# MarSaKi/VLN-BEVBert

Measured on AMD Instinct MI355X. Metric: pretrain_samples_per_sec, higher is better.
Workload: dtype bf16+fp32-residual

## Files before the change

### include/bevbert_hip.h

```cpp
#ifndef BEVBERT_HIP_H
#define BEVBERT_HIP_H

#include <stdint.h>

#ifdef __cplusplus
extern "C" {
#endif

typedef struct ihipStream_t* hipStream_t;

#define BEVBERT_F32 0
#define BEVBERT_BF16 1
#define BEVBERT_F16 2

const char* bevbert_last_error(void);
int bevbert_version(void);
int bevbert_hip_error_reset(void);
const char* bevbert_arch(void);
const char* bevbert_attn_last_path(int backward);

int bevbert_bev_lift_bin(const float* depths, const float* T_c2w, const float* T_w2c, const float* S_w2c,
                         const float* pix_scale, int B, int V, int hw, float depth_scale, int dim, float res,
                         float y_clip, int* cell, int* order, int* cell_start, hipStream_t stream);
int bevbert_bev_bin_points(const float* points, const uint8_t* drop_mask, int B, int P, int dim, float res,
// ... 35 lines not shown
                                const float* gamma, const float* beta, void* y16, float* y32, float* z32, float* mean,
                                float* rstd, int rows, int H, float eps, float drop_p, uint64_t seed, uint64_t offset,
                                hipStream_t stream);
int bevbert_layernorm_res32_bwd(const void* dy16, const float* dy32, const float* z32, const float* mean,
                                const float* rstd, const float* gamma, void* dz, void* dx16, float* dgamma,
                                float* dbeta, float* dbias, float* workspace, int rows, int H, float drop_p, uint64_t seed,
                                uint64_t offset, int accumulate, int dz_dtype,
                                hipStream_t stream);
int64_t bevbert_colsum_workspace_floats(int total_cols);
int bevbert_colsum_partial_rows(int rows);
int bevbert_colsum_finalize(const float* partials, int nblocks, int nwhich, int C, float* out0, float* out1,
                            float* out2, int accumulate, hipStream_t stream);
int bevbert_colsum_partials(const void* dy, float* partials, int rows, int C, int dtype, hipStream_t stream);
int bevbert_multi_finalize(const void* tasks, int ntasks, hipStream_t stream);
int bevbert_multi_accum(const void* tasks, int ntasks, hipStream_t stream);

int bevbert_embed_sum_layernorm_fwd(const int64_t* ids, const void* word, const void* pos, const void* type_row,
                                    const float* gamma, const float* beta, void* y, void* z_out, float* mean,
                                    float* rstd, int rows, int L, int H, float eps, int dtype, float drop_p,
                                    uint64_t seed, uint64_t offset, hipStream_t stream);

int bevbert_embedding_grad(const int64_t* ids, const void* d, float* table_grad, int rows, int H, int padding_idx,
                           int dtype, hipStream_t stream);

int64_t bevbert_smallk_workspace_floats(int rows, int K, int H);
int bevbert_smallk_linear_layernorm_fwd(const float* feat, const float* weight, const float* bias, const float* gamma,
                                        const float* beta, const void* post1, const void* table, const int64_t* idx,
                                        void* y, float* mean, float* rstd, int rows, int K, int H, float eps, int dtype,
                                        hipStream_t stream);
int bevbert_smallk_linear_layernorm_bwd(const void* dy, const float* feat, const float* weight, const float* bias,
// ... 28 lines not shown

int bevbert_bias_gelu_fwd(const void* x, const float* bias, void* y, int rows, int C, int dtype, hipStream_t stream);
int bevbert_bias_gelu_bwd(const void* dy, const void* x, const float* bias, void* dx, float* dbias, float* workspace,
                          int rows, int C, int dtype, int accumulate, hipStream_t stream);
int bevbert_bias_relu_fwd(const void* x, const float* bias, void* y, int rows, int C, int dtype, hipStream_t stream);
int bevbert_bias_relu_bwd(const void* dy, const void* x, const float* bias, void* dx, float* dbias, float* workspace,
                          int rows, int C, int dtype, int accumulate, hipStream_t stream);
int bevbert_colsum(const void* dy, float* out, float* workspace, int rows, int C, int dtype, int accumulate,
                   hipStream_t stream);

int bevbert_segment_wsum(const void* src, const int* rowptr, const int* idx, const float* w, void* out, int out_rows,
                         int H, int dtype, hipStream_t stream);

int bevbert_grad_norm_clip(const float* grads, int64_t n, float pre_scale, float max_norm, float* partials,
                           float* scalars, hipStream_t stream);
int bevbert_adamw_step(float* params, const float* grads, float* exp_avg, float* exp_avg_sq, void* params_bf16,
                       const uint8_t* chunk_flags, int* chunk_steps, int64_t n, const float* grad_scale_dev,
                       const float* lr_dev, float lr, float beta1, float beta2, float eps, float weight_decay,
                       hipStream_t stream);
int bevbert_cast_f32(const float* src, void* dst, int64_t n, int dst_dtype, hipStream_t stream);
int bevbert_zero(void* p, int64_t bytes, hipStream_t stream);
int bevbert_accum_partials(const void* partials, float* sink, int S, int64_t n, int dtype, hipStream_t stream);

int bevbert_gemm(const void* A, const void* B, void* C, const void* bias, int M, int N, int K, int opA, int opB,
                 int64_t lda, int64_t ldb, int64_t ldc, int batch, int64_t stride_a, int64_t stride_b,
                 int64_t stride_c, int in_dtype, int out_dtype, int bias_dtype, float alpha, void* workspace,
                 int64_t workspace_bytes, int autotune, hipStream_t stream);
int bevbert_gemm_plan(int M, int N, int K, int opA, int opB, int64_t lda, int64_t ldb, int64_t ldc, int batch,
                      int64_t stride_a, int64_t stride_b, int64_t stride_c, int in_dtype, int out_dtype, int bias_dtype,
                      int accumulate, int64_t workspace_bytes, int autotune);
// ... 95 lines not shown
```

### vln_bevbert_amd/arena.py

```python
import math

import torch

from . import lib
from .lib import ptr, stream


def call(name, *args):
    from . import ops
    return ops.call(name, *args)

CHUNK = 1024
_ZERO_KERNEL = __import__("os").environ.get("BEVBERT_ZERO_KERNEL", "0") == "1"
NO_DECAY = ("bias", "LayerNorm.bias", "LayerNorm.weight")


def _round_up(n, m):
    return (n + m - 1) // m * m


class ParamArena:
    def __init__(self, module, device, compute_dtype=torch.float32, groups=()):
        self.device = torch.device(device)
        self.compute_dtype = compute_dtype
# ... 42 lines not shown
                self._flags_host[start // CHUNK:end // CHUNK] |= 1
            for n in seg:
                self._seg_of[n] = (start // CHUNK, end // CHUNK)
        self.flags = self._flags_host.to(dev)
        self.chunk_steps = torch.zeros(off // CHUNK, dtype=torch.int32, device=dev)
        self._touched = set()
        self._flags_dirty = False
        self.publish_grads = True
        self.allreduce_group = None
        self.defer_allreduce = False
        self._cb_queued = False
        self._fresh = []
        self._published = []
        self._param_versions = None
        self.step_count = 0
        self._scalars = torch.zeros(4, dtype=torch.float32, device=dev)
        self._partials = torch.zeros(1024, dtype=torch.float32, device=dev)
        self.named = named
        for n, p in named:
            o, k = self.slices[n]
            view = self.params[o:o + k].view(p.shape)
            view.copy_(p.data.to(dev, torch.float32))
            p.data = view
            p.main_grad = self.grads[o:o + k].view(p.shape)
            p.compute = self.shadow[o:o + k].view(p.shape) if self.shadow is not None else p.data
            p.arena = self
            p.arena_name = n
        self._index = {n: i for i, (n, _) in enumerate(named)}
        self.sync_shadow()
        self._param_versions = sum(p._version for _, p in named)

    def packed(self, names, shape):
        o0, _ = self.slices[names[0]]
        total = 0
        for n in names:
            o, k = self.slices[n]
            assert o == o0 + total, f"{names} are not contiguous in the arena"
            total += k
        assert total == math.prod(shape)
        src = self.shadow if self.shadow is not None else self.params
        return src[o0:o0 + total].view(shape), self.grads[o0:o0 + total].view(shape)

    def touch(self, param):
        n = param.arena_name
        if n not in self._touched:
            self._touched.add(n)
            a, b = self._seg_of[n]
            self._flags_host[a:b] |= 2
            self._flags_dirty = True
        if self.publish_grads:
            self._note_backward_write(param)

    def _note_backward_write(self, param):
        if not self._cb_queued:
            try:
                torch.autograd.Variable._execution_engine.queue_callback(self._publish)
            except RuntimeError:
                return
            self._cb_queued = True
# ... 48 lines not shown

    def sync(self):
        if self.device.type == "cuda":
            from . import ops
            ops.WgradStream.flush_all()
            cur = torch.cuda.current_stream(self.device)
            for side in ops.Branches.side_streams():
                if ops.Branches.enabled or side not in ops.WgradStream.streams or ops.WgradStream.dirty:
                    cur.wait_stream(side)
            ops.WgradStream.dirty = False
            ops.WgradStream.release()

    def backward_done(self):
        self.sync()

    def zero_grad(self, overlap=False):
        self.sync()
        if self.device.type == "cuda":
            from . import ops
            ops.RT.scratch.reset()
            if overlap:
                if getattr(self, "_zero_stream", None) is None:
                    from .hwqueues import side_stream
                    self._zero_stream = side_stream(self.device)
                self._zero_stream.wait_stream(torch.cuda.current_stream(self.device))
                with torch.cuda.stream(self._zero_stream):
                    if _ZERO_KERNEL:
                        self.grads.zero_()
                    else:
                        call("bevbert_zero", ptr(self.grads), self.grads.numel() * 4, stream())
                self._zero_pending = True
                return
            call("bevbert_zero", ptr(self.grads), self.grads.numel() * 4, stream())
            return
        self.grads.zero_()

    def wait_zero(self):
        if getattr(self, "_zero_pending", False):
            torch.cuda.current_stream(self.device).wait_stream(self._zero_stream)
            self._zero_pending = False

    def load_state_dict_into(self, module, sd, strict=True):
        out = module.load_state_dict(sd, strict=strict)
        self.sync_shadow()
        return out

    def set_lr(self, lr):
        self._scalars[2:3].fill_(float(lr))
        self._lr_set = True

    def upload_flags(self):
        if self._flags_dirty:
            self.flags.copy_(self._flags_host, non_blocking=True)
            self._flags_dirty = False

    def clip_and_step(self, lr=None, betas=(0.9, 0.98), eps=1e-6, weight_decay=0.01, max_norm=5.0, grad_pre_scale=1.0):
        self.sync()
        if self.exp_avg is None:
            self.exp_avg = torch.zeros_like(self.params)
            self.exp_avg_sq = torch.zeros_like(self.params)
        if lr is not None:
            self.set_lr(lr)
        elif not getattr(self, "_lr_set", False):
            raise RuntimeError("clip_and_step(lr=None) reads the device-resident learning rate: call set_lr() first "
                               "(the slot starts at 0, which would silently turn AdamW and its weight decay into a no-op)")
        if not torch.cuda.is_current_stream_capturing():
            self.upload_flags()
        self.step_count += 1
        call("bevbert_grad_norm_clip", ptr(self.grads), self.numel, float(grad_pre_scale),
             float(max_norm if max_norm is not None else -1.0), ptr(self._partials), ptr(self._scalars), stream())
        call("bevbert_adamw_step", ptr(self.params), ptr(self.grads), ptr(self.exp_avg), ptr(self.exp_avg_sq),
             ptr(self.shadow), ptr(self.flags), ptr(self.chunk_steps), self.numel, self._scalars[1:].data_ptr(),
             self._scalars[2:].data_ptr(), 0.0, float(betas[0]), float(betas[1]), float(eps), float(weight_decay),
             stream())

    def grad_norm(self):
        return self._scalars[0]
```

### vln_bevbert_amd/csrc/capi.hip

```cpp
#include <stdarg.h>

#include "attn_common.h"

static thread_local char g_err[512] = "";

void bb_set_error(const char* fmt, ...) {
  va_list ap;
  va_start(ap, fmt);
  vsnprintf(g_err, sizeof(g_err), fmt, ap);
  va_end(ap);
}

BEVBERT_API const char* bevbert_last_error(void) { return g_err; }
BEVBERT_API int bevbert_hip_error_reset(void) {
  int n = 0;
  while (hipGetLastError() != hipSuccess && n < 16) ++n;
  return n;
}

BEVBERT_API int bevbert_zero(void* p, int64_t bytes, hipStream_t stream) {
  BB_REQUIRE(p != nullptr && bytes >= 0, "zero: null pointer or negative size");
  if (bytes == 0) return BB_OK;
  hipError_t e = hipMemsetAsync(p, 0, (size_t)bytes, stream);
  if (e != hipSuccess) {
    bb_set_error("zero: hipMemsetAsync failed: %s", hipGetErrorString(e));
    return BB_ELAUNCH;
  }
  return BB_OK;
}

BEVBERT_API int bevbert_version(void) { return 112; }

static const uint32_t* g_step_salt = nullptr;
const uint32_t* bb_step_salt() { return g_step_salt; }
BEVBERT_API int bevbert_set_step_salt(const void* device_word) {
  g_step_salt = static_cast<const uint32_t*>(device_word);
  return BB_OK;
}
BEVBERT_API const char* bevbert_arch(void) { return "gfx950"; }

int attn_simple_fwd(const AttnArgs& a, int dtype, hipStream_t st);
int attn_simple_bwd(const AttnArgs& a, int dtype, hipStream_t st);
int attn_delta(const AttnArgs& a, float* delta, int dtype, hipStream_t st);
int attn_mfma_fwd(const AttnArgs& a, hipStream_t st);
int attn_mfma_bwd(const AttnArgs& a, hipStream_t st);
int attn_mfma_bwd1(const AttnArgs& a, hipStream_t st);
// ... 166 lines not shown
```

### vln_bevbert_amd/csrc/rowops.hip

```cpp
#include <math.h>

#include "common.h"

template <typename T, int NV, bool GATHER>
__global__ __launch_bounds__(256) void ln_fwd_kernel(const T* __restrict__ x, const float* __restrict__ bias,
                                                     const T* __restrict__ residual, const float* __restrict__ gamma,
                                                     const float* __restrict__ beta, T* __restrict__ y,
                                                     T* __restrict__ z_out, float* __restrict__ mean_out,
                                                     float* __restrict__ rstd_out, int rows, float eps, float drop_p,
                                                     uint32_t drop_thr, uint32_t drop_key,
                                                     const int64_t* __restrict__ ids, const T* __restrict__ word,
                                                     const T* __restrict__ pos, const T* __restrict__ type_row, int L,
                                                     const uint32_t* __restrict__ salt) {
  constexpr int H = NV * 256;
  if (drop_p > 0.f) drop_key = bb_salted(drop_key, salt);
  const int lane = threadIdx.x & 63;
  const int row = blockIdx.x * 4 + (threadIdx.x >> 6);
  if (row >= rows) return;
  float4 v[NV];
  const float keep_scale = drop_p > 0.f ? 1.0f / (1.0f - drop_p) : 1.0f;
#pragma unroll
  for (int i = 0; i < NV; ++i) {
    const int col = (i * 64 + lane) * 4;
    float4 a;
// ... 502 lines not shown
  for (unsigned i = threadIdx.x; i < t.n4; i += 256) {
    float4 acc = *reinterpret_cast<const float4*>(t.sink + (size_t)i * 4);
    for (int s = 0; s < t.S; ++s) {
      const float4 v = ld4<T>(part + ((size_t)s * t.n4_total + t.off4 + i) * 4);
      acc.x += v.x; acc.y += v.y; acc.z += v.z; acc.w += v.w;
    }
    *reinterpret_cast<float4*>(t.sink + (size_t)i * 4) = acc;
  }
}
__global__ __launch_bounds__(256) void multi_accum_kernel(const AccumTask* __restrict__ tasks) {
  const AccumTask t = tasks[blockIdx.x];
  if (t.dtype == BB_BF16) accum_task<bf16_raw>(t);
  else accum_task<float>(t);
}

#define EG_MAXJ 4
template <typename T, typename TO = float, bool ACCUM = true>
__global__ __launch_bounds__(256) void embedding_grad_kernel(const int64_t* __restrict__ ids, const T* __restrict__ d,
                                                             TO* __restrict__ table_grad, int rows, int H,
                                                             int padding_idx) {
  __shared__ int s_flag;
  __shared__ float s_part[4][256 * EG_MAXJ];
  const int r = blockIdx.x, tid = threadIdx.x, lane = tid & 63, wave = tid >> 6;
  const int64_t id = ids[r];
  if (id == (int64_t)padding_idx) return;
  if (tid == 0) s_flag = 0;
  __syncthreads();
  int hit = 0;
  for (int i = tid; i < r; i += 256) hit |= (ids[i] == id);
  if (hit) s_flag = 1;
// ... 79 lines not shown
    const float4 v = *reinterpret_cast<const float4*>(g + i * 4);
    s += (v.x * v.x + v.y * v.y) + (v.z * v.z + v.w * v.w);
  }
  __shared__ float sh[4];
  s = wave_sum(s);
  if ((threadIdx.x & 63) == 0) sh[threadIdx.x >> 6] = s;
  __syncthreads();
  if (threadIdx.x == 0) partials[blockIdx.x] = (sh[0] + sh[1]) + (sh[2] + sh[3]);
}

__global__ void clip_coef_kernel(const float* __restrict__ partials, int n, float pre_scale, float max_norm,
                                 float* __restrict__ scalars) {
  __shared__ double sh[256];
  double s = 0.0;
  for (int i = threadIdx.x; i < n; i += 256) s += (double)partials[i];
  sh[threadIdx.x] = s;
  __syncthreads();
  for (int o = 128; o > 0; o >>= 1) {
    if (threadIdx.x < o) sh[threadIdx.x] += sh[threadIdx.x + o];
    __syncthreads();
  }
  if (threadIdx.x == 0) {
    const float norm = (float)sqrt(sh[0]) * pre_scale;
    float coef = 1.0f;
    if (max_norm > 0.f) {
      coef = max_norm / (norm + 1e-6f);
      coef = coef < 1.0f ? coef : 1.0f;
    }
    scalars[0] = norm;
    scalars[1] = pre_scale * coef;
// ... 659 lines not shown
    return BB_EUNSUPPORTED;
  }
  BB_CHECK_LAUNCH("colsum_partials");
  return BB_OK;
}

BEVBERT_API int bevbert_multi_accum(const void* tasks, int ntasks, hipStream_t stream) {
  static_assert(sizeof(AccumTask) == 40, "AccumTask is part of the C ABI");
  if (ntasks <= 0) return BB_OK;
  BB_REQUIRE(tasks != nullptr, "multi_accum: null task table");
  hipLaunchKernelGGL(multi_accum_kernel, dim3(ntasks), dim3(256), 0, stream, (const AccumTask*)tasks);
  BB_CHECK_LAUNCH("multi_accum");
  return BB_OK;
}

BEVBERT_API int bevbert_multi_finalize(const void* tasks, int ntasks, hipStream_t stream) {
  static_assert(sizeof(FinalizeTask) == 40, "FinalizeTask is part of the C ABI");
  if (ntasks <= 0) return BB_OK;
  BB_REQUIRE(tasks != nullptr, "multi_finalize: null task table");
  hipLaunchKernelGGL(multi_finalize_kernel, dim3(ntasks), dim3(64, 16), 0, stream, (const FinalizeTask*)tasks);
  BB_CHECK_LAUNCH("multi_finalize");
  return BB_OK;
}

BEVBERT_API int bevbert_segment_wsum(const void* src, const int* rowptr, const int* idx, const float* w, void* out,
                                     int out_rows, int H, int dtype, hipStream_t stream) {
  BB_REQUIRE(H % 4 == 0, "segment_wsum: H=%d must be a multiple of 4", H);
  if (out_rows <= 0) return BB_OK;
  if (dtype == BB_F32)
    hipLaunchKernelGGL(gather_wsum_kernel<float>, dim3(out_rows), dim3(192), 0, stream, (const float*)src, rowptr, idx, w, (float*)out, H);
// ... 97 lines not shown
                       rows, H, rows_per_slice, table_rows);
  else {
    bb_set_error("embedding_grad_sliced: dtype %d unsupported", dtype);
    return BB_EUNSUPPORTED;
  }
  BB_CHECK_LAUNCH("embedding_grad_sliced");
  return BB_OK;
}

BEVBERT_API int bevbert_grad_norm_clip(const float* grads, int64_t n, float pre_scale, float max_norm,
                                       float* partials, float* scalars, hipStream_t stream) {
  BB_REQUIRE(n % 4 == 0, "grad_norm_clip: n must be a multiple of 4");
  hipLaunchKernelGGL(sumsq_kernel, dim3(1024), dim3(256), 0, stream, grads, (size_t)n / 4, partials);
  hipLaunchKernelGGL(clip_coef_kernel, dim3(1), dim3(256), 0, stream, partials, 1024, pre_scale, max_norm, scalars);
  BB_CHECK_LAUNCH("grad_norm_clip");
  return BB_OK;
}

BEVBERT_API int bevbert_adamw_step(float* params, const float* grads, float* exp_avg, float* exp_avg_sq,
                                   void* params_bf16, const uint8_t* chunk_flags, int* chunk_steps, int64_t n,
                                   const float* grad_scale_dev, const float* lr_dev, float lr, float beta1,
                                   float beta2, float eps, float weight_decay, hipStream_t stream) {
  BB_REQUIRE(n % 1024 == 0, "adamw_step: arena length must be a multiple of 1024 elements");
  BB_REQUIRE(chunk_steps != nullptr, "adamw_step: per-chunk step counters are required");
  const size_t nchunks = (size_t)n / 1024;
  hipLaunchKernelGGL(adamw_kernel, dim3(nchunks), dim3(256), 0, stream, params, grads, exp_avg, exp_avg_sq,
                     (bf16_raw*)params_bf16, chunk_flags, chunk_steps, nchunks, grad_scale_dev, lr_dev, lr, beta1, beta2, eps,
                     weight_decay, (float)log2((double)beta1), (float)log2((double)beta2));
  BB_CHECK_LAUNCH("adamw_step");
  return BB_OK;
// ... 45 lines not shown
```

### vln_bevbert_amd/lib.py

```python
import ctypes
import os
import re
import subprocess

import torch

_HERE = os.path.dirname(os.path.abspath(__file__))
LIB_PATH = os.path.join(_HERE, "libbevbert_hip.so")
CSRC = os.path.join(_HERE, "csrc")
EXTRA_FLAGS = {"attn_fwd4.hip": ["-fno-slp-vectorize"]}
SOURCES = ["splat.hip", "rowops.hip", "attn_simple.hip", "attn_f32.hip", "attn_mfma.hip", "attn_bwd1.hip", "attn_fwd2.hip", "attn_fwd4.hip", "attn_bwd2.hip", "attn_bwd3.hip", "attn_small.hip", "attn_short.hip", "smallk.hip", "sap_loss.hip", "graph_nav.hip", "nav_expert.hip", "gemm.hip", "capi.hip"]
HEADER = os.path.join(os.path.dirname(_HERE), "include", "bevbert_hip.h")

F32, BF16, F16 = 0, 1, 2
_DT = {torch.float32: F32, torch.bfloat16: BF16, torch.float16: F16}


class BevBertHipError(RuntimeError):
    pass


def dtype_code(t):
    try:
        return _DT[t.dtype if torch.is_tensor(t) else t]
# ... 67 lines not shown
    "bevbert_smallk_linear_layernorm_bwd": [_P] * 12 + [_I, _I, _I, _I, _P],
    "bevbert_rows_scatter": [_P, _P, _P, _I, _I, _I, _I, _P],
    "bevbert_embedding_grad_sliced": [_P, _P, _P, _I, _I, _I, _I, _I, _P],
    "bevbert_bias_gelu_fwd": [_P, _P, _P, _I, _I, _I, _P],
    "bevbert_bias_gelu_bwd": [_P, _P, _P, _P, _P, _P, _I, _I, _I, _I, _P],
    "bevbert_bias_relu_fwd": [_P, _P, _P, _I, _I, _I, _P],
    "bevbert_bias_relu_bwd": [_P, _P, _P, _P, _P, _P, _I, _I, _I, _I, _P],
    "bevbert_colsum": [_P, _P, _P, _I, _I, _I, _I, _P],
    "bevbert_segment_wsum": [_P, _P, _P, _P, _P, _I, _I, _I, _P],
    "bevbert_grad_norm_clip": [_P, _I64, _F, _F, _P, _P, _P],
    "bevbert_adamw_step": [_P, _P, _P, _P, _P, _P, _P, _I64, _P, _P, _F, _F, _F, _F, _F, _P],
    "bevbert_set_step_salt": [_P],
    "bevbert_colsum_partials": [_P, _P, _I, _I, _I, _P],
    "bevbert_multi_finalize": [_P, _I, _P],
    "bevbert_multi_accum": [_P, _I, _P],
    "bevbert_cast_f32": [_P, _P, _I64, _I, _P],
    "bevbert_zero": [_P, _I64, _P],
    "bevbert_accum_partials": [_P, _P, _I, _I64, _I, _P],
    "bevbert_dropout_keep_mask": [_P, _I64, _F, _U64, _U64, _P],
    "bevbert_gemm": [_P, _P, _P, _P, _I, _I, _I, _I, _I, _I64, _I64, _I64, _I, _I64, _I64, _I64, _I, _I, _I, _F, _P,
                     _I64, _I, _P],
    "bevbert_colsum_finalize": [_P, _I, _I, _I, _P, _P, _P, _I, _P],
    "bevbert_dropout_add": [_P, _P, _P, _I64, _I, _I, _F, _U64, _U64, _P],
    "bevbert_gm_update": [_P] * 10 + [_I, _I, _P, _P, _P],
    "bevbert_gm_nav_vars": [_P] * 7 + [_I, _I, _I] + [_P] * 7,
    "bevbert_gm_bev_select": [_P, _P, _I, _I, _P, _P, _P, _P, _P],
    "bevbert_gm_gather_views": [_P, _P, _P, _P, _I, _I64, _P],
    "bevbert_gm_embed_update": [_P] * 9 + [_I, _I, _I, _I, _P],
    "bevbert_gm_node_embeds": [_P, _P, _P, _P, _P, _I, _I, _I, _P, _P],
    "bevbert_sap_loss_fwd": [_P] * 15 + [_I, _I, _I, _I, _I, _P],
# ... 94 lines not shown
```

### vln_bevbert_amd/ops_reduce.py

```python
import math
import os as _os

import torch

from . import lib
from .lib import stream
from .ops_core import ATTN_BITS, Branches, RT, call


def join_captured_side_streams(extra=()):
    if not torch.cuda.is_available() or not torch.cuda.is_current_stream_capturing():
        return 0
    cur = torch.cuda.current_stream()
    seen, n = {cur.cuda_stream}, 0
    cands = [ATTN_BITS.stream] + list(Branches._streams.values()) + list(WgradStream.streams) + list(extra)
    for st in cands:
        if st is None or st.cuda_stream in seen:
            continue
        seen.add(st.cuda_stream)
        with torch.cuda.stream(st):
            capturing = torch.cuda.is_current_stream_capturing()
        if capturing:
            cur.wait_stream(st)
            n += 1
# ... 182 lines not shown

ScratchRing.INITIAL = int(_os.environ.get("BEVBERT_SCRATCH_INITIAL_MB", "256")) << 20
RT.scratch = SCRATCH


class ReduceQueue:

    jobs = []
    accum_jobs = []
    table_bytes = {}
    producers = {}
    _tables = {}
    _accum_tables = {}
    _dtype = None
    _adtype = None

    @classmethod
    def _note_producer(cls):
        st = WgradStream._target
        if st is None:
            if not torch.cuda.is_available():
                return
            st = torch.cuda.current_stream()
        cls.producers[st.cuda_stream] = st

    @classmethod
    def wait_producers(cls, consumer):
        for h, st in cls.producers.items():
            if h != consumer.cuda_stream:
                consumer.wait_stream(st)
        cls.producers = {}

    @classmethod
    def drop_pending(cls):
        cls.jobs, cls.accum_jobs, cls.producers = [], [], {}

    @classmethod
    def add_accum(cls, partials_ptr, sink_ptr, S, n, dtype):
        cls.accum_jobs.append((partials_ptr, sink_ptr, S, n, dtype))
        cls._note_producer()

    @classmethod
    def _build_accum(cls, jobs, device):
        import numpy as np
        if cls._adtype is None:
            cls._adtype = np.dtype([("partials", "<u8"), ("sink", "<u8"), ("n4_total", "<u8"), ("off4", "<u4"),
                                    ("n4", "<u4"), ("S", "<i4"), ("dtype", "<i4")])
        parts = []
        for partials_ptr, sink_ptr, S, n, dt in jobs:
            n4 = n // 4
            off = np.arange(0, n4, 4096, dtype=np.int64)
            t = np.zeros(len(off), dtype=cls._adtype)
            t["partials"] = partials_ptr
            t["sink"] = sink_ptr + off * 16
            t["n4_total"] = n4
            t["off4"] = off
            t["n4"] = np.minimum(4096, n4 - off)
            t["S"] = S
            t["dtype"] = dt
            parts.append(t)
        table = np.concatenate(parts) if parts else np.zeros(0, dtype=cls._adtype)
        dev = torch.from_numpy(table.view(np.uint8).copy()).to(device)
        cls.table_bytes[dev.data_ptr()] = int(sum(S * n * (4 if dt == lib.F32 else 2) + 8 * n for _, _, S, n, dt in jobs))
        return dev, len(table)

    @classmethod
    def add(cls, partials_ptr, nblocks, nwhich, C, outs, accumulate=1):
        cls.jobs.append((partials_ptr, nblocks, nwhich, C, outs[0] or 0, outs[1] or 0, outs[2] or 0, accumulate))
        cls._note_producer()

    @classmethod
    def _build(cls, jobs, device):
        import numpy as np
        if cls._dtype is None:
            cls._dtype = np.dtype([("partials", "<u8"), ("out", "<u8"), ("nblocks", "<i4"), ("row_stride", "<i4"),
                                   ("col0", "<i4"), ("ncols", "<i4"), ("accumulate", "<i4"), ("pad", "<i4")])
        parts = []
        for partials_ptr, nblocks, nwhich, C, o0, o1, o2, acc in jobs:
            ntile = (C + 63) // 64
# ... 6 lines not shown
                t["out"] = out + tiles * 256
                t["nblocks"] = nblocks
                t["row_stride"] = nwhich * C
                t["col0"] = which * C + tiles * 64
                t["ncols"] = np.minimum(64, C - tiles * 64)
                t["accumulate"] = acc
                parts.append(t)
        table = np.concatenate(parts) if parts else np.zeros(0, dtype=cls._dtype)
        dev = torch.from_numpy(table.view(np.uint8).copy()).to(device)
        cls.table_bytes[dev.data_ptr()] = int(4 * (table["nblocks"].astype(np.int64) * table["ncols"]).sum()
                                              + 4 * (table["ncols"] * (1 + (table["accumulate"] != 0))).sum()) if len(table) else 0
        return dev, len(table)

    @classmethod
    def flush(cls, device):
        if cls.accum_jobs:
            akey = tuple(cls.accum_jobs)
            cls.accum_jobs = []
            aent = cls._accum_tables.get(akey)
            if aent is None:
                if torch.cuda.is_current_stream_capturing():
                    raise lib.BevBertHipError("accumulate task table missing during graph capture (warm-up steps build it)")
                if len(cls._accum_tables) > 256:
                    cls._accum_tables.clear()
                rounds, seen = [[]], [set()]
                for job in akey:
                    r = 0
                    while job[1] in seen[r]:
                        r += 1
                        if r == len(rounds):
                            rounds.append([])
# ... 48 lines not shown
```

### vln_bevbert_amd/train.py

```python
import os
import random

import torch
import torch.distributed as dist

from . import ops
from .static_step import GraphedStep, StaticBatch


def warmup_linear_lr(step, base_lr, warmup_steps, total_steps):
    f = step / warmup_steps if step < warmup_steps else max(0, (total_steps - step) / (total_steps - warmup_steps))
    lr = base_lr * f
    return lr if lr > 0 else 1e-8


def load_gemm_tuning():
    import os
    path = os.path.join(os.path.dirname(os.path.abspath(__file__)), "tunableop_results.csv")
    if os.environ.get("BEVBERT_GEMM_TUNING", "1") != "1" or not os.path.exists(path):
        return 0
    try:
        import torch.cuda.tunable as tunable
        tunable.enable(True)
        tunable.tuning_enable(False)
# ... 215 lines not shown
        first_map = min(arena.slices[n][0] for n in arena.slices
                        if n.startswith("bert.local_encoder") or n.startswith("bert.global_encoder")
                        or not n.startswith("bert."))
        self.reducer = GradReducer(arena.grads, first_map, force=force_collectives)
        self.reducer.set_occupied(arena.slices.values())
        self.reducer.settle_collective_queue()
        self.overlap = overlap and self.reducer.active
        self.capture_ok = not (self.reducer.active and self.reducer.exchange == "bf16_a2a")
        if self.reducer.active and dist.get_backend(self.reducer.group) != "nccl":
            self.capture_ok = False
        if self.reducer.active:
            self.broadcast_state()
        self.early_flush = os.environ.get("BEVBERT_EARLY_FLUSH", "0") == "1" and arena.device.type == "cuda"
        if self.early_flush and not self.overlap:
            model.bert.lang_encoder.register_forward_hook(self._hook_flush)
        if self.overlap:
            self.install_map_layer_hooks()
            model.bert.lang_encoder.register_forward_hook(self._hook_text)
            for k, lo, hi in self.text_layer_regions(model, arena):
                model.bert.lang_encoder.layer[k].register_forward_pre_hook(self._make_layer_hook(lo, hi))

    @staticmethod
    def map_layer_regions(model, arena):
        out = {}
        heads = [(o, o + k) for n, (o, k) in arena.slices.items() if not n.startswith("bert.")]
        if heads:
            lo, hi = min(lo for lo, _ in heads), max(hi for _, hi in heads)
            if not any(n.startswith("bert.") and lo <= o < hi for n, (o, c) in arena.slices.items()):
                out["heads"] = (lo, hi)
        for enc in ("local", "global"):
# ... 85 lines not shown

    def _step_seed(self):
        return (self.seed + self.rank) * 1000003 + self.global_step

    def forward_backward(self, task, batch):
        self.global_step += 1
        ops.RT.new_step(self._step_seed(), plan_key=self._plan_key(task, batch))
        return self._forward_backward(task, batch)

    @staticmethod
    def _plan_key(task, batch):
        return (task, batch.signature) if isinstance(batch, StaticBatch) else None

    def _forward_backward(self, task, batch):
        self._reset_map_hooks()
        self.arena.zero_grad(overlap=self.overlap_zero)
        try:
            if isinstance(batch, StaticBatch):
                loss = self.model.loss_mean(batch.tensors, task)
            else:
                loss = self.model(batch, task, compute_loss=True).mean()
        finally:
            self.arena.wait_zero()
        if self.reducer is not None and self.reducer.timeline is not None:
            self.backward_start = torch.cuda.Event(enable_timing=True)
            self.backward_start.record()
        if loss.is_cuda and loss.dim() == 0:
            one = self.__dict__.get("_one")
            if one is None or one.dtype != loss.dtype or one.device != loss.device:
                one = self._one = torch.ones((), dtype=loss.dtype, device=loss.device)
            loss.backward(gradient=one)
        else:
            loss.backward()
        self.arena.sync()
        self.reducer.finish()
        return loss.detach()

    def optimizer_step(self, lr=None):
        if lr is None:
            lr = warmup_linear_lr(self.global_step, self.lr, self.warmup, self.total)
        self.arena.clip_and_step(lr, self.betas, 1e-6, self.wd, self.grad_norm, grad_pre_scale=1.0 / self.world)

    def step(self, task, batch):
        if isinstance(batch, StaticBatch) and self.use_graphs and self.capture_ok and batch.capturable and ops.RT.trace is None:
            return self._static_step(task, batch)
        loss = self.forward_backward(task, batch)
        self.optimizer_step()
        return loss

    GRAPH_WARMUP = 2

    def _static_step(self, task, sb):
        assert sb.task == task
        self.global_step += 1
        lr = warmup_linear_lr(self.global_step, self.lr, self.warmup, self.total)
        a = self.arena
# ... 22 lines not shown
        torch.cuda.synchronize()
        graph = torch.cuda.CUDAGraph()
        if self._graph_pool is None:
            self._graph_pool = torch.cuda.graph_pool_handle()
        ops.Branches.enabled = branches or self.graph_branches
        mode = "thread_local"
        if self.reducer.active:
            import time
            time.sleep(0.3)
        err = None
        try:
            with torch.cuda.graph(graph, pool=self._graph_pool, capture_error_mode=mode):
                try:
                    ops.RT.new_step(0, write_salt=False, plan_key=self._plan_key(task, sb))
                    loss = self._forward_backward(task, sb)
                    a.clip_and_step(None, self.betas, 1e-6, self.wd, self.grad_norm, grad_pre_scale=1.0 / self.world)
                except Exception as e:
                    err = e
                    ops.join_captured_side_streams(extra=[self.reducer.stream])
        except Exception as e:
            err = err or e
        if err is not None:
            e = err
            import warnings
            self.graph_error = f"{type(e).__name__}: {e}"[:400]
            self.use_graphs = False
            warnings.warn(f"hipGraph capture of the {task} step failed, continuing with eager steps: {self.graph_error}")
            ops.Branches.enabled = branches
            from . import lib
            lib.load().bevbert_hip_error_reset()
            if torch.cuda.is_current_stream_capturing():
# ... 60 lines not shown
```

Measured before the change: 3552.

## Fold grad accumulation into assignment and fuse grad-norm partials into the fold

After: 3599 (median of 6 runs). 1.01x the previous value.

```diff
diff --git a/include/bevbert_hip.h b/include/bevbert_hip.h
--- a/include/bevbert_hip.h
+++ b/include/bevbert_hip.h
@@ -73,6 +73,7 @@
 int bevbert_colsum_partials(const void* dy, float* partials, int rows, int C, int dtype, hipStream_t stream);
 int bevbert_multi_finalize(const void* tasks, int ntasks, hipStream_t stream);
 int bevbert_multi_accum(const void* tasks, int ntasks, hipStream_t stream);
+int bevbert_multi_accum2(const void* tasks, int ntasks, float* sumsq_out, hipStream_t stream);
 
 int bevbert_embed_sum_layernorm_fwd(const int64_t* ids, const void* word, const void* pos, const void* type_row,
                                     const float* gamma, const float* beta, void* y, void* z_out, float* mean,
@@ -131,6 +132,11 @@
 
 int bevbert_grad_norm_clip(const float* grads, int64_t n, float pre_scale, float max_norm, float* partials,
                            float* scalars, hipStream_t stream);
+int bevbert_grad_sumsq_ranges(const float* grads, const void* ranges, int nranges, float* partials_out,
+                              hipStream_t stream);
+int bevbert_zero_ranges(float* grads, const void* ranges, int nranges, hipStream_t stream);
+int bevbert_clip_coef2(const float* sumsq_a, int na, const float* sumsq_b, int nb, float pre_scale, float max_norm,
+                       float* scalars, hipStream_t stream);
 int bevbert_adamw_step(float* params, const float* grads, float* exp_avg, float* exp_avg_sq, void* params_bf16,
                        const uint8_t* chunk_flags, int* chunk_steps, int64_t n, const float* grad_scale_dev,
                        const float* lr_dev, float lr, float beta1, float beta2, float eps, float weight_decay,
diff --git a/vln_bevbert_amd/arena.py b/vln_bevbert_amd/arena.py
--- a/vln_bevbert_amd/arena.py
+++ b/vln_bevbert_amd/arena.py
@@ -80,6 +80,16 @@
         self._published = []
         self._param_versions = None
         self.step_count = 0
+        self.assign_fold = False
+        self._assign_pass = False
+        self._fold_excluded = set()
+        self._touch_count = {}
+        self._fold_plans = {}
+        self._fold_key = None
+        self._fold_state = None
+        self._unzeroed = ()
+        self._range_tables = {}
+        self._slice_starts = None
         self._scalars = torch.zeros(4, dtype=torch.float32, device=dev)
         self._partials = torch.zeros(1024, dtype=torch.float32, device=dev)
         self.named = named
@@ -109,6 +119,8 @@
 
     def touch(self, param):
         n = param.arena_name
+        if self._assign_pass:
+            self._touch_count[n] = self._touch_count.get(n, 0) + 1
         if n not in self._touched:
             self._touched.add(n)
             a, b = self._seg_of[n]
@@ -187,26 +199,124 @@
     def backward_done(self):
         self.sync()
 
-    def zero_grad(self, overlap=False):
+    def zero_grad(self, overlap=False, fold_key=None, assign=False):
         self.sync()
+        self._fold_state = None
+        self._assign_pass = assign = bool(assign) and self.assign_fold
+        self._fold_key = fold_key if assign else None
+        stored = self._fold_plans.get(fold_key) if self._fold_key is not None else None
+        self._unzeroed = stored or ()
+        if assign:
+            self._touch_count.clear()
         if self.device.type == "cuda":
             from . import ops
             ops.RT.scratch.reset()
+            ops.ReduceQueue.begin_pass(self if assign else None)
             if overlap:
                 if getattr(self, "_zero_stream", None) is None:
                     from .hwqueues import side_stream
                     self._zero_stream = side_stream(self.device)
                 self._zero_stream.wait_stream(torch.cuda.current_stream(self.device))
                 with torch.cuda.stream(self._zero_stream):
-                    if _ZERO_KERNEL:
+                    if stored:
+                        self._fill_complement(stored)
+                    elif _ZERO_KERNEL:
                         self.grads.zero_()
                     else:
                         call("bevbert_zero", ptr(self.grads), self.grads.numel() * 4, stream())
                 self._zero_pending = True
                 return
-            call("bevbert_zero", ptr(self.grads), self.grads.numel() * 4, stream())
+            if stored:
+                self._fill_complement(stored)
+            else:
+                call("bevbert_zero", ptr(self.grads), self.grads.numel() * 4, stream())
             return
         self.grads.zero_()
+
+    FOLD_PIECE = 16384
+    MAX_MEMSETS = 16
+
+    def enable_assign_fold(self, module, on=True):
+        self.assign_fold = bool(on) and self.device.type == "cuda"
+        self._fold_state = None
+        if not on:
+            return
+        tables = {id(m.weight) for m in module.modules() if isinstance(m, torch.nn.Embedding)}
+        self._fold_excluded = {n for n, p in self.named if p.dim() != 2 or id(p) in tables or p.shape[1] <= 16}
+        order = sorted((o, k, n) for n, (o, k) in self.slices.items())
+        self._slice_starts = ([o for o, _, _ in order], order)
+
+    def owns_grad_ptr(self, p):
+        return 0 <= p - self.grads.data_ptr() < 4 * self.numel
+
+    def fold_store_flags(self, jobs):
+        import bisect
+        base, starts, order = self.grads.data_ptr(), self._slice_starts[0], self._slice_starts[1]
+        spans = []
+        for _, sink, _, n, _ in jobs:
+            off = (sink - base) // 4
+            spans.append((off, off + n) if (sink - base) % 4 == 0 and 0 <= off and off + n <= self.numel else None)
+        flags, stored = [], []
+        for j, span in enumerate(spans):
+            ok = span is not None and span[0] % CHUNK == 0
+            if ok:
+                lo, hi = span
+                ok = not any(o is not None and i != j and o[0] < _round_up(hi, CHUNK) and lo < o[1]
+                             for i, o in enumerate(spans))
+            if ok:
+                i = bisect.bisect_left(starts, lo)
+                pos, ok = lo, i < len(order) and order[i][0] == lo
+                while ok and pos < hi:
+                    if i == len(order) or order[i][0] != pos:
+                        ok = False
+                        break
+                    o, k, name = order[i]
+                    ok = name not in self._fold_excluded and self._touch_count.get(name, 0) == 1
+                    pos, i = o + k, i + 1
+                ok = ok and pos == hi and (i == len(order) or order[i][0] >= _round_up(hi, CHUNK))
+            flags.append(bool(ok))
+            if ok:
+                stored.append((lo, _round_up(hi, CHUNK)))
+        return tuple(flags), tuple(sorted(stored))
+
+    def fold_ranges(self, stored):
+        ent = self._range_tables.get(stored)
+        if ent is None:
+            if self.device.type == "cuda" and torch.cuda.is_current_stream_capturing():
+                raise lib.BevBertHipError("arena range table missing during graph capture (warm-up steps build it)")
+            if len(self._range_tables) > 64:
+                self._range_tables.clear()
+            merged, pos = [], 0
+            for lo, hi in stored:
+                if lo > pos:
+                    merged.append((pos, lo))
+                pos = max(pos, hi)
+            if pos < self.numel:
+                merged.append((pos, self.numel))
+            pieces = [(a, min(self.FOLD_PIECE, hi - a)) for lo, hi in merged for a in range(lo, hi, self.FOLD_PIECE)]
+            table = torch.tensor(pieces, dtype=torch.int64).reshape(-1, 2).to(self.device)
+            ent = self._range_tables[stored] = {"merged": merged, "table": table, "n": len(pieces),
+                                                "partials": torch.zeros(max(len(pieces), 1), dtype=torch.float32,
+                                                                        device=self.device)}
+        return ent
+
+    def _fill_complement(self, stored):
+        ent = self.fold_ranges(stored)
+        if len(ent["merged"]) <= self.MAX_MEMSETS:
+            for lo, hi in ent["merged"]:
+                call("bevbert_zero", ptr(self.grads) + 4 * lo, 4 * (hi - lo), stream())
+        else:
+            call("bevbert_zero_ranges", ptr(self.grads), ptr(ent["table"]), ent["n"], stream())
+
+    def note_fold(self, stored, sumsq, nstore):
+        if not set(self._unzeroed) <= set(stored):
+            raise lib.BevBertHipError("assign-fold: the step's fill skipped arena ranges its fold did not store "
+                                      f"(plan key {self._fold_key!r} no longer describes the backward pass)")
+        if self._fold_key is not None:
+            if len(self._fold_plans) > 256:
+                self._fold_plans.clear()
+            self._fold_plans[self._fold_key] = stored
+        self._fold_state = (sumsq, nstore, self.fold_ranges(stored))
 
     def wait_zero(self):
         if getattr(self, "_zero_pending", False):
@@ -227,7 +337,8 @@
             self.flags.copy_(self._flags_host, non_blocking=True)
             self._flags_dirty = False
 
-    def clip_and_step(self, lr=None, betas=(0.9, 0.98), eps=1e-6, weight_decay=0.01, max_norm=5.0, grad_pre_scale=1.0):
+    def clip_and_step(self, lr=None, betas=(0.9, 0.98), eps=1e-6, weight_decay=0.01, max_norm=5.0, grad_pre_scale=1.0,
+                      fused_norm=False):
         self.sync()
         if self.exp_avg is None:
             self.exp_avg = torch.zeros_like(self.params)
@@ -240,8 +351,15 @@
         if not torch.cuda.is_current_stream_capturing():
             self.upload_flags()
         self.step_count += 1
-        call("bevbert_grad_norm_clip", ptr(self.grads), self.numel, float(grad_pre_scale),
-             float(max_norm if max_norm is not None else -1.0), ptr(self._partials), ptr(self._scalars), stream())
+        fold, self._fold_state = self._fold_state, None
+        if fused_norm and fold is not None:
+            sumsq, nstore, rt = fold
+            call("bevbert_grad_sumsq_ranges", ptr(self.grads), ptr(rt["table"]), rt["n"], ptr(rt["partials"]), stream())
+            call("bevbert_clip_coef2", ptr(sumsq), nstore, ptr(rt["partials"]), rt["n"], float(grad_pre_scale),
+                 float(max_norm if max_norm is not None else -1.0), ptr(self._scalars), stream())
+        else:
+            call("bevbert_grad_norm_clip", ptr(self.grads), self.numel, float(grad_pre_scale),
+                 float(max_norm if max_norm is not None else -1.0), ptr(self._partials), ptr(self._scalars), stream())
         call("bevbert_adamw_step", ptr(self.params), ptr(self.grads), ptr(self.exp_avg), ptr(self.exp_avg_sq),
              ptr(self.shadow), ptr(self.flags), ptr(self.chunk_steps), self.numel, self._scalars[1:].data_ptr(),
              self._scalars[2:].data_ptr(), 0.0, float(betas[0]), float(betas[1]), float(eps), float(weight_decay),
diff --git a/vln_bevbert_amd/csrc/capi.hip b/vln_bevbert_amd/csrc/capi.hip
--- a/vln_bevbert_amd/csrc/capi.hip
+++ b/vln_bevbert_amd/csrc/capi.hip
@@ -29,7 +29,7 @@
   return BB_OK;
 }
 
-BEVBERT_API int bevbert_version(void) { return 112; }
+BEVBERT_API int bevbert_version(void) { return 113; }
 
 static const uint32_t* g_step_salt = nullptr;
 const uint32_t* bb_step_salt() { return g_step_salt; }
diff --git a/vln_bevbert_amd/csrc/rowops.hip b/vln_bevbert_amd/csrc/rowops.hip
--- a/vln_bevbert_amd/csrc/rowops.hip
+++ b/vln_bevbert_amd/csrc/rowops.hip
@@ -540,6 +540,64 @@
   else accum_task<float>(t);
 }
 
+struct AccumTask2 {
+  const void* partials;
+  float* sink;
+  unsigned long long n4_total;
+  unsigned int off4, n4;
+  int S, dtype;
+  int store, pad;
+};
+template <typename T, bool STORE>
+__device__ __forceinline__ float accum_task2(const AccumTask2& t) {
+  const T* part = (const T*)t.partials + (size_t)t.off4 * 4;
+  const size_t slice = (size_t)t.n4_total * 4;
+  float sq = 0.f;
+  for (unsigned base = threadIdx.x; base < t.n4; base += 1024) {
+    float4 acc[4];
+    bool ok[4];
+#pragma unroll
+    for (int u = 0; u < 4; ++u) {
+      const unsigned i = base + u * 256;
+      ok[u] = i < t.n4;
+      acc[u] = make_float4(0.f, 0.f, 0.f, 0.f);
+      if (!STORE && ok[u]) acc[u] = *reinterpret_cast<const float4*>(t.sink + (size_t)i * 4);
+    }
+    for (int s = 0; s < t.S; ++s) {
+      float4 v[4];
+#pragma unroll
+      for (int u = 0; u < 4; ++u) {
+        const unsigned i = base + u * 256;
+        v[u] = ok[u] ? ld4<T>(part + (size_t)s * slice + (size_t)i * 4) : make_float4(0.f, 0.f, 0.f, 0.f);
+      }
+#pragma unroll
+      for (int u = 0; u < 4; ++u) {
+        acc[u].x += v[u].x; acc[u].y += v[u].y; acc[u].z += v[u].z; acc[u].w += v[u].w;
+      }
+    }
+#pragma unroll
+    for (int u = 0; u < 4; ++u) {
+      if (ok[u]) {
+        *reinterpret_cast<float4*>(t.sink + (size_t)(base + u * 256) * 4) = acc[u];
+        sq += (acc[u].x * acc[u].x + acc[u].y * acc[u].y) + (acc[u].z * acc[u].z + acc[u].w * acc[u].w);
+      }
+    }
+  }
+  return sq;
+}
+__global__ __launch_bounds__(256) void multi_accum2_kernel(const AccumTask2* __restrict__ tasks,
+                                                           float* __restrict__ sumsq_out) {
+  const AccumTask2 t = tasks[blockIdx.x];
+  float sq;
+  if (t.store) sq = t.dtype == BB_BF16 ? accum_task2<bf16_raw, true>(t) : accum_task2<float, true>(t);
+  else sq = t.dtype == BB_BF16 ? accum_task2<bf16_raw, false>(t) : accum_task2<float, false>(t);
+  __shared__ float sh[4];
+  sq = wave_sum(sq);
+  if ((threadIdx.x & 63) == 0) sh[threadIdx.x >> 6] = sq;
+  __syncthreads();
+  if (threadIdx.x == 0) sumsq_out[blockIdx.x] = (sh[0] + sh[1]) + (sh[2] + sh[3]);
+}
+
 #define EG_MAXJ 4
 template <typename T, typename TO = float, bool ACCUM = true>
 __global__ __launch_bounds__(256) void embedding_grad_kernel(const int64_t* __restrict__ ids, const T* __restrict__ d,
@@ -649,6 +707,64 @@
   __shared__ double sh[256];
   double s = 0.0;
   for (int i = threadIdx.x; i < n; i += 256) s += (double)partials[i];
+  sh[threadIdx.x] = s;
+  __syncthreads();
+  for (int o = 128; o > 0; o >>= 1) {
+    if (threadIdx.x < o) sh[threadIdx.x] += sh[threadIdx.x + o];
+    __syncthreads();
+  }
+  if (threadIdx.x == 0) {
+    const float norm = (float)sqrt(sh[0]) * pre_scale;
+    float coef = 1.0f;
+    if (max_norm > 0.f) {
+      coef = max_norm / (norm + 1e-6f);
+      coef = coef < 1.0f ? coef : 1.0f;
+    }
+    scalars[0] = norm;
+    scalars[1] = pre_scale * coef;
+  }
+}
+
+struct ArenaRange { long long start, count; };
+__global__ __launch_bounds__(256) void sumsq_ranges_kernel(const float* __restrict__ g, const ArenaRange* __restrict__ ranges,
+                                                           float* __restrict__ partials) {
+  const ArenaRange r = ranges[blockIdx.x];
+  const float* p = g + r.start;
+  const size_t n4 = (size_t)r.count / 4;
+  float s = 0.f;
+  size_t i = threadIdx.x;
+  for (; i + 768 < n4; i += 1024) {
+    float4 v[4];
+#pragma unroll
+    for (int u = 0; u < 4; ++u) v[u] = *reinterpret_cast<const float4*>(p + (i + u * 256) * 4);
+#pragma unroll
+    for (int u = 0; u < 4; ++u) s += (v[u].x * v[u].x + v[u].y * v[u].y) + (v[u].z * v[u].z + v[u].w * v[u].w);
+  }
+  for (; i < n4; i += 256) {
+    const float4 v = *reinterpret_cast<const float4*>(p + i * 4);
+    s += (v.x * v.x + v.y * v.y) + (v.z * v.z + v.w * v.w);
+  }
+  __shared__ float sh[4];
+  s = wave_sum(s);
+  if ((threadIdx.x & 63) == 0) sh[threadIdx.x >> 6] = s;
+  __syncthreads();
+  if (threadIdx.x == 0) partials[blockIdx.x] = (sh[0] + sh[1]) + (sh[2] + sh[3]);
+}
+
+__global__ __launch_bounds__(256) void zero_ranges_kernel(float* __restrict__ g, const ArenaRange* __restrict__ ranges) {
+  const ArenaRange r = ranges[blockIdx.x];
+  float* p = g + r.start;
+  const size_t n4 = (size_t)r.count / 4;
+  const float4 z = make_float4(0.f, 0.f, 0.f, 0.f);
+  for (size_t i = threadIdx.x; i < n4; i += 256) *reinterpret_cast<float4*>(p + i * 4) = z;
+}
+
+__global__ void clip_coef2_kernel(const float* __restrict__ pa, int na, const float* __restrict__ pb, int nb,
+                                  float pre_scale, float max_norm, float* __restrict__ scalars) {
+  __shared__ double sh[256];
+  double s = 0.0;
+  for (int i = threadIdx.x; i < na; i += 256) s += (double)pa[i];
+  for (int i = threadIdx.x; i < nb; i += 256) s += (double)pb[i];
   sh[threadIdx.x] = s;
   __syncthreads();
   for (int o = 128; o > 0; o >>= 1) {
@@ -1338,6 +1454,15 @@
   return BB_OK;
 }
 
+BEVBERT_API int bevbert_multi_accum2(const void* tasks, int ntasks, float* sumsq_out, hipStream_t stream) {
+  static_assert(sizeof(AccumTask2) == 48, "AccumTask2 is part of the C ABI");
+  if (ntasks <= 0) return BB_OK;
+  BB_REQUIRE(tasks != nullptr && sumsq_out != nullptr, "multi_accum2: null task table or sumsq_out");
+  hipLaunchKernelGGL(multi_accum2_kernel, dim3(ntasks), dim3(256), 0, stream, (const AccumTask2*)tasks, sumsq_out);
+  BB_CHECK_LAUNCH("multi_accum2");
+  return BB_OK;
+}
+
 BEVBERT_API int bevbert_multi_finalize(const void* tasks, int ntasks, hipStream_t stream) {
   static_assert(sizeof(FinalizeTask) == 40, "FinalizeTask is part of the C ABI");
   if (ntasks <= 0) return BB_OK;
@@ -1465,6 +1590,33 @@
   hipLaunchKernelGGL(sumsq_kernel, dim3(1024), dim3(256), 0, stream, grads, (size_t)n / 4, partials);
   hipLaunchKernelGGL(clip_coef_kernel, dim3(1), dim3(256), 0, stream, partials, 1024, pre_scale, max_norm, scalars);
   BB_CHECK_LAUNCH("grad_norm_clip");
+  return BB_OK;
+}
+
+BEVBERT_API int bevbert_grad_sumsq_ranges(const float* grads, const void* ranges, int nranges, float* partials_out,
+                                          hipStream_t stream) {
+  static_assert(sizeof(ArenaRange) == 16, "ArenaRange is part of the C ABI");
+  if (nranges <= 0) return BB_OK;
+  BB_REQUIRE(grads != nullptr && ranges != nullptr && partials_out != nullptr, "grad_sumsq_ranges: null pointer");
+  hipLaunchKernelGGL(sumsq_ranges_kernel, dim3(nranges), dim3(256), 0, stream, grads, (const ArenaRange*)ranges, partials_out);
+  BB_CHECK_LAUNCH("grad_sumsq_ranges");
+  return BB_OK;
+}
+
+BEVBERT_API int bevbert_zero_ranges(float* grads, const void* ranges, int nranges, hipStream_t stream) {
+  if (nranges <= 0) return BB_OK;
+  BB_REQUIRE(grads != nullptr && ranges != nullptr, "zero_ranges: null pointer");
+  hipLaunchKernelGGL(zero_ranges_kernel, dim3(nranges), dim3(256), 0, stream, grads, (const ArenaRange*)ranges);
+  BB_CHECK_LAUNCH("zero_ranges");
+  return BB_OK;
+}
+
+BEVBERT_API int bevbert_clip_coef2(const float* sumsq_a, int na, const float* sumsq_b, int nb, float pre_scale,
+                                   float max_norm, float* scalars, hipStream_t stream) {
+  BB_REQUIRE(na >= 0 && nb >= 0 && scalars != nullptr && (na == 0 || sumsq_a) && (nb == 0 || sumsq_b),
+             "clip_coef2: bad arguments");
+  hipLaunchKernelGGL(clip_coef2_kernel, dim3(1), dim3(256), 0, stream, sumsq_a, na, sumsq_b, nb, pre_scale, max_norm, scalars);
+  BB_CHECK_LAUNCH("clip_coef2");
   return BB_OK;
 }
 
diff --git a/vln_bevbert_amd/lib.py b/vln_bevbert_amd/lib.py
--- a/vln_bevbert_amd/lib.py
+++ b/vln_bevbert_amd/lib.py
@@ -105,6 +105,10 @@
     "bevbert_colsum_partials": [_P, _P, _I, _I, _I, _P],
     "bevbert_multi_finalize": [_P, _I, _P],
     "bevbert_multi_accum": [_P, _I, _P],
+    "bevbert_multi_accum2": [_P, _I, _P, _P],
+    "bevbert_grad_sumsq_ranges": [_P, _P, _I, _P, _P],
+    "bevbert_zero_ranges": [_P, _P, _I, _P],
+    "bevbert_clip_coef2": [_P, _I, _P, _I, _F, _F, _P, _P],
     "bevbert_cast_f32": [_P, _P, _I64, _I, _P],
     "bevbert_zero": [_P, _I64, _P],
     "bevbert_accum_partials": [_P, _P, _I, _I64, _I, _P],
diff --git a/vln_bevbert_amd/ops_reduce.py b/vln_bevbert_amd/ops_reduce.py
--- a/vln_bevbert_amd/ops_reduce.py
+++ b/vln_bevbert_amd/ops_reduce.py
@@ -220,6 +220,10 @@
     _accum_tables = {}
     _dtype = None
     _adtype = None
+    _adtype2 = None
+    assign_arena = None
+    _assigned = None
+    _assign_tables = {}
 
     @classmethod
     def _note_producer(cls):
@@ -240,6 +244,12 @@
     @classmethod
     def drop_pending(cls):
         cls.jobs, cls.accum_jobs, cls.producers = [], [], {}
+        cls.assign_arena = cls._assigned = None
+
+    @classmethod
+    def begin_pass(cls, arena):
+        import weakref
+        cls.assign_arena, cls._assigned = (weakref.ref(arena) if arena is not None else None), None
 
     @classmethod
     def add_accum(cls, partials_ptr, sink_ptr, S, n, dtype):
@@ -269,6 +279,70 @@
         dev = torch.from_numpy(table.view(np.uint8).copy()).to(device)
         cls.table_bytes[dev.data_ptr()] = int(sum(S * n * (4 if dt == lib.F32 else 2) + 8 * n for _, _, S, n, dt in jobs))
         return dev, len(table)
+
+    @classmethod
+    def _build_accum2(cls, jobs, store, device):
+        import numpy as np
+        if cls._adtype2 is None:
+            cls._adtype2 = np.dtype([("partials", "<u8"), ("sink", "<u8"), ("n4_total", "<u8"), ("off4", "<u4"),
+                                     ("n4", "<u4"), ("S", "<i4"), ("dtype", "<i4"), ("store", "<i4"), ("pad", "<i4")])
+        parts = []
+        for (partials_ptr, sink_ptr, S, n, dt), st in zip(jobs, store):
+            n4 = n // 4
+            off = np.arange(0, n4, 4096, dtype=np.int64)
+            t = np.zeros(len(off), dtype=cls._adtype2)
+            t["partials"] = partials_ptr
+            t["sink"] = sink_ptr + off * 16
+            t["n4_total"] = n4
+            t["off4"] = off
+            t["n4"] = np.minimum(4096, n4 - off)
+            t["S"] = S
+            t["dtype"] = dt
+            t["store"] = int(st)
+            parts.append(t)
+        table = np.concatenate(parts) if parts else np.zeros(0, dtype=cls._adtype2)
+        dev = torch.from_numpy(table.view(np.uint8).copy()).to(device)
+        cls.table_bytes[dev.data_ptr()] = int(sum(S * n * (4 if dt == lib.F32 else 2) + (4 if st else 8) * n
+                                                  for (_, _, S, n, dt), st in zip(jobs, store)))
+        return dev, len(table), int(sum(len(t) for t, st in zip(parts, store) if st))
+
+    @classmethod
+    def _flush_assign(cls, arena, device):
+        akey = tuple(cls.accum_jobs)
+        cls.accum_jobs = []
+        key = (akey, id(arena), tuple(arena._touch_count.items()))
+        ent = cls._assign_tables.get(key)
+        if ent is None:
+            if torch.cuda.is_current_stream_capturing():
+                raise lib.BevBertHipError("accumulate task table missing during graph capture (warm-up steps build it)")
+            if len(cls._assign_tables) > 256:
+                cls._assign_tables.clear()
+            flags, stored = arena.fold_store_flags(akey)
+            rounds, rflags, seen = [[j for j, f in zip(akey, flags) if f]], [[]], [set()]
+            rflags[0] = [True] * len(rounds[0])
+            seen[0] = {j[1] for j in rounds[0]}
+            for job in (j for j, f in zip(akey, flags) if not f):
+                r = 0
+                while job[1] in seen[r]:
+                    r += 1
+                    if r == len(rounds):
+                        rounds.append([])
+                        rflags.append([])
+                        seen.append(set())
+                rounds[r].append(job)
+                rflags[r].append(False)
+                seen[r].add(job[1])
+            tables = [cls._build_accum2(tuple(r), tuple(f), device) for r, f in zip(rounds, rflags)]
+            sumsq = torch.empty(max(1, sum(n for _, n, _ in tables)), dtype=torch.float32, device=device)
+            ent = cls._assign_tables[key] = (tables, sumsq, tables[0][2], stored)
+        tables, sumsq, nstore, stored = ent
+        off = 0
+        for table, n, _ in tables:
+            call("bevbert_multi_accum2", table.data_ptr(), n, sumsq.data_ptr() + 4 * off, stream())
+            off += n
+        import weakref
+        cls._assigned = weakref.ref(arena)
+        arena.note_fold(stored, sumsq, nstore)
 
     @classmethod
     def add(cls, partials_ptr, nblocks, nwhich, C, outs, accumulate=1):
@@ -305,7 +379,15 @@
 
     @classmethod
     def flush(cls, device):
-        if cls.accum_jobs:
+        arena = cls.assign_arena() if cls.assign_arena is not None else None
+        if cls.accum_jobs and arena is not None:
+            cls.assign_arena = None
+            cls._flush_assign(arena, device)
+        elif cls.accum_jobs:
+            done = cls._assigned() if cls._assigned is not None else None
+            if done is not None and done._fold_state is not None and any(done.owns_grad_ptr(j[1]) for j in cls.accum_jobs):
+                raise lib.BevBertHipError("assign-fold mode folds once per backward pass: a second fold would accumulate "
+                                          "onto ranges whose norm has been taken (turn the mode off for this loop)")
             akey = tuple(cls.accum_jobs)
             cls.accum_jobs = []
             aent = cls._accum_tables.get(akey)
diff --git a/vln_bevbert_amd/train.py b/vln_bevbert_amd/train.py
--- a/vln_bevbert_amd/train.py
+++ b/vln_bevbert_amd/train.py
@@ -253,6 +253,8 @@
         self.early_flush = os.environ.get("BEVBERT_EARLY_FLUSH", "0") == "1" and arena.device.type == "cuda"
         if self.early_flush and not self.overlap:
             model.bert.lang_encoder.register_forward_hook(self._hook_flush)
+        arena.enable_assign_fold(model, os.environ.get("BEVBERT_ASSIGN_FOLD", "1") == "1" and not self.reducer.active
+                                 and not self.early_flush and ops.WgradStream.DEFER_FINALIZE)
         if self.overlap:
             self.install_map_layer_hooks()
             model.bert.lang_encoder.register_forward_hook(self._hook_text)
@@ -368,7 +370,7 @@
 
     def _forward_backward(self, task, batch):
         self._reset_map_hooks()
-        self.arena.zero_grad(overlap=self.overlap_zero)
+        self.arena.zero_grad(overlap=self.overlap_zero, fold_key=self._plan_key(task, batch), assign=True)
         try:
             if isinstance(batch, StaticBatch):
                 loss = self.model.loss_mean(batch.tensors, task)
@@ -393,7 +395,8 @@
     def optimizer_step(self, lr=None):
         if lr is None:
             lr = warmup_linear_lr(self.global_step, self.lr, self.warmup, self.total)
-        self.arena.clip_and_step(lr, self.betas, 1e-6, self.wd, self.grad_norm, grad_pre_scale=1.0 / self.world)
+        self.arena.clip_and_step(lr, self.betas, 1e-6, self.wd, self.grad_norm, grad_pre_scale=1.0 / self.world,
+                                 fused_norm=True)
 
     def step(self, task, batch):
         if isinstance(batch, StaticBatch) and self.use_graphs and self.capture_ok and batch.capturable and ops.RT.trace is None:
@@ -446,7 +449,8 @@
                 try:
                     ops.RT.new_step(0, write_salt=False, plan_key=self._plan_key(task, sb))
                     loss = self._forward_backward(task, sb)
-                    a.clip_and_step(None, self.betas, 1e-6, self.wd, self.grad_norm, grad_pre_scale=1.0 / self.world)
+                    a.clip_and_step(None, self.betas, 1e-6, self.wd, self.grad_norm, grad_pre_scale=1.0 / self.world,
+                                    fused_norm=True)
                 except Exception as e:
                     err = e
                     ops.join_captured_side_streams(extra=[self.reducer.stream])
```
